# yuansliu/minicom

Measured on AMD Instinct MI355X. Metric: Mreads/s (sketch+index+overlap) on 150bp reads, 1/2/4/8 GPU; bit-exact decompress, higher is better.
Workload: dtype u64

## Files before the change

minicom_amd/csrc/api.hip:

```cpp
#include "mcom_dev.hpp"
#include "../../include/mcom_test.h"
#include <stdarg.h>
#include <stdlib.h>
#include <cxxabi.h>
#include <stdio.h>
#include <string.h>

int mcom_fail(mcom_ctx *ctx, int code, const char *fmt, ...)
{
	char buf[512];
	va_list ap;
	va_start(ap, fmt);
	vsnprintf(buf, sizeof buf, fmt, ap);
	va_end(ap);
	if (ctx) { ctx->err = buf; ctx->pin_wait.clear(); ctx->pin_off = 0; }
	return code;
}

#define MCOM_PIN_BYTES 4096
hipError_t mcom_d2h_async(mcom_ctx *ctx, void *dst, const void *src, size_t bytes)
{
	for (uint32_t q = 0; q < 8; ++q) {
		const mcom_ctx::ScanTotal &t = ctx->scan_last[(ctx->scan_last_at + 7u - q) % 8u];
		if (t.last && t.last == src && t.bytes == bytes && t.gen == ctx->launch_gen) { mcom_ctx::PinWait w{dst, 0, bytes}; w.from = ctx->scan_tot + t.slot; ctx->pin_wait.push_back(w); return hipSuccess; }
// ... 257 lines not shown
extern "C" int mcom_prof_kernels(mcom_ctx *ctx, const char *name, char *buf, size_t cap, size_t *need)
{
	if (!ctx || !name) return MCOM_E_ARG;
	int cls = -1;
	if (!strcmp(name, "*")) cls = -2;
	else if (!strcmp(name, "-")) cls = PROF_COUNT;
	else for (int i = 0; i < PROF_COUNT; ++i) if (!strcmp(name, PROF_NAMES[i])) cls = i;
	if (cls == -1) return mcom_fail(ctx, MCOM_E_ARG, "unknown profiler name %s", name);
	std::map<std::string, uint64_t> out;
	for (const auto &kv : ctx->prof_kernels) if (cls == -2 || kv.first.first == cls) out[prof_kernel_text(ctx, kv.first.second)] += kv.second;
	std::string txt;
	for (const auto &kv : out) { txt += kv.first; txt += '\t'; txt += std::to_string(kv.second); txt += '\n'; }
	if (need) *need = txt.size() + 1;
	if (buf && cap) { size_t m = txt.size() < cap - 1 ? txt.size() : cap - 1; memcpy(buf, txt.data(), m); buf[m] = 0; }
	return MCOM_OK;
}

extern "C" int mcom_prof_read(mcom_ctx *ctx, const char *name, double *total_ms, uint64_t *launches)
{
	if (!ctx || !name) return MCOM_E_ARG;
	prof_collect(ctx);
	for (int i = 0; i < PROF_COUNT; ++i) if (!strcmp(name, PROF_NAMES[i])) {
		if (total_ms) *total_ms = ctx->prof_ms[i];
		if (launches) *launches = ctx->prof_calls[i];
		return MCOM_OK;
	}
	return mcom_fail(ctx, MCOM_E_ARG, "unknown profiler name %s", name);
}

extern "C" uint64_t mcom_counter(const mcom_ctx *ctx, const char *name)
{
	if (!ctx || !name) return 0;
	if (!strcmp(name, "sort_overflow_segments")) return ctx->sort_overflow_segments;
	if (!strcmp(name, "sketch_strings")) return ctx->sketch_strings;
	return 0;
}
extern "C" int mcom_set_segment_capacity(mcom_ctx *ctx, uint32_t records)
{
	if (!ctx || records > 4096) return MCOM_E_ARG;
	ctx->seg_cap = records;
	return MCOM_OK;
}
extern "C" int mcom_set_consensus_capacity(mcom_ctx *ctx, uint32_t members)
{
	if (!ctx) return MCOM_E_ARG;
	ctx->bs_cap = members;
	return MCOM_OK;
}
extern "C" int mcom_set_sketch_kernel(mcom_ctx *ctx, int wave_per_string)
{
	if (!ctx) return MCOM_E_ARG;
	ctx->sketch_wave_only = wave_per_string == 1;
	ctx->sketch_ring64 = wave_per_string == 2;
	ctx->sketch_ring32_only = wave_per_string == 3;
	ctx->sketch_lane_always = wave_per_string >= 2;
	return MCOM_OK;
}
extern "C" int mcom_set_sketch_prefix_bits(mcom_ctx *ctx, int bits)
{
	if (!ctx || bits < 1 || bits > 30) return MCOM_E_ARG;
	ctx->sketch_prefix_bits = bits;
	return MCOM_OK;
}
extern "C" int mcom_set_claim_route(mcom_ctx *ctx, int route)
{
	if (!ctx || route < 0 || route > 3) return MCOM_E_ARG;
	ctx->claim_route = route;
	return MCOM_OK;
}
extern "C" int mcom_claim_fallbacks(const mcom_ctx *ctx) { return ctx ? (int)ctx->claim_fallbacks : 0; }
extern "C" int mcom_set_screen_route(mcom_ctx *ctx, int route)
{
	if (!ctx || route < 0 || route > 2) return MCOM_E_ARG;
	ctx->screen_route = route;
	return MCOM_OK;
}
extern "C" int mcom_screen_fallbacks(const mcom_ctx *ctx) { return ctx ? (int)ctx->screen_fallbacks : 0; }
extern "C" int mcom_set_lookup_route(mcom_ctx *ctx, int route)
{
	if (!ctx || route < 0 || route > 1) return MCOM_E_ARG;
	ctx->lookup_route = route;
	return MCOM_OK;
}
extern "C" int mcom_set_index_capacity(mcom_ctx *ctx, int entries)
{
	if (!ctx) return MCOM_E_ARG;
	ctx->cix_cap_set = entries >= 0; ctx->cix_cap = entries >= 0 ? (uint32_t)entries : 0u;
	return MCOM_OK;
}
```

minicom_amd/csrc/contigs.hip:

```cpp
#include "mcom_dev.hpp"
#include <cstring>
#include <cstdlib>
#include <algorithm>
#include <vector>

#define MAXW 128

__device__ __forceinline__ int nt4_of(uint8_t ch)
{
	const uint8_t u = ch & 0xDF;
	return u == 'A' ? 0 : u == 'C' ? 1 : u == 'G' ? 2 : u == 'T' ? 3 : 4;
}

#define PIECE 128
#define NGRP (PIECE / 64)
#define ERING 256
#define EMASK (ERING - 1)
#define RBCAP 64

__device__ __forceinline__ uint64_t rev_groups64(uint64_t x)
{
	x = __brevll(x);
	return ((x >> 1) & 0x5555555555555555ull) | ((x & 0x5555555555555555ull) << 1);
}
// ... 786 lines not shown
}
__global__ void k_fn_qcounts(const uint32_t *__restrict__ roff, const uint32_t *__restrict__ ord, size_t n, uint32_t *__restrict__ cnt)
{
	const size_t u = (size_t)blockIdx.x * blockDim.x + threadIdx.x;
	if (u > n) return;
	if (u == n) { cnt[u] = 0; return; }
	const uint32_t c = ord ? ord[u] : (uint32_t)u;
	cnt[u] = roff[c + 1] - roff[c];
}
__global__ __launch_bounds__(256) void k_fn_counts_ord(const uint64_t *__restrict__ slots, uint32_t log2cap, uint32_t region, uint32_t bbits,
                                                       const mcom_mm128 *__restrict__ rec, const uint32_t *__restrict__ roff, const uint32_t *__restrict__ ord,
                                                       const uint32_t *__restrict__ qoff, size_t n, uint32_t nq, uint32_t new_lo, uint32_t new_span, int kbits,
                                                       const uint32_t *__restrict__ keymap, uint32_t *__restrict__ hits, uint32_t *__restrict__ first,
                                                       uint64_t *__restrict__ qy)
{
	const size_t u = ((size_t)blockIdx.x * blockDim.x + threadIdx.x) >> 4;
	if (u >= n) return;
	const int lane = threadIdx.x & 15;
	if (u == 0 && lane == 0) hits[nq] = 0;
	const uint32_t c = ord ? ord[u] : (uint32_t)u;
	const uint32_t r0 = roff[c], cnt = roff[c + 1] - r0, q0 = qoff[u];
	const bool old_contig = new_span && !fn_is_new(c, new_lo, new_span);
	for (uint32_t t0 = lane; t0 < cnt; t0 += 64) {
		mcom_mm128 v[4];
#pragma unroll
		for (int u = 0; u < 4; ++u) { const uint32_t t = t0 + 16u * u; if (t < cnt) v[u] = rec[r0 + t]; else { v[u].x = U64MAX; v[u].y = 0; } }
		bool look[4];
#pragma unroll
		for (int u = 0; u < 4; ++u) {
			look[u] = v[u].x != U64MAX;
			if (look[u] && old_contig) { const uint32_t h = fn_key_bit(v[u].x, kbits); look[u] = (keymap[h >> 5] >> (h & 31)) & 1u; }
		}
#pragma unroll
		for (int u = 0; u < 4; ++u) {
			const uint32_t t = t0 + 16u * u;
			if (t >= cnt) break;
			uint32_t s = 0, k = 0;
			if (look[u]) mcom_table_find_any(slots, log2cap, region, bbits, v[u].x, s, k);
			hits[q0 + t] = k;
			if (k) { first[q0 + t] = s; qy[q0 + t] = v[u].y; }
		}
	}
}
__global__ void k_fn_expand(const uint32_t *__restrict__ pair_off, size_t nq, uint32_t *__restrict__ pair_q)
{
	const size_t i = (size_t)blockIdx.x * blockDim.x + threadIdx.x;
	if (i >= nq) return;
	const uint32_t p0 = pair_off[i], p1 = pair_off[i + 1];
	for (uint32_t p = p0; p < p1; ++p) pair_q[p] = (uint32_t)i;
}
__global__ void k_fn_eval(const uint32_t *__restrict__ first, const mcom_mm128 *__restrict__ irec,
                          const mcom_mm128 *__restrict__ q, const uint64_t *__restrict__ qy, const uint32_t *__restrict__ pair_off, const uint32_t *__restrict__ pair_q, uint32_t n_pairs,
                          const uint64_t *__restrict__ cbits, const uint64_t *__restrict__ coff, const uint32_t *__restrict__ clen,
                          int cbthr, uint32_t new_lo, uint32_t new_span, uint32_t *__restrict__ pass)
{
	const uint32_t p = blockIdx.x * blockDim.x + threadIdx.x;
	if (p >= n_pairs) return;
	const uint32_t i = pair_q[p];
	const uint32_t u = p - pair_off[i], s = first[i];
	const uint64_t my = qy ? qy[i] : q[i].y, y = irec[s + u].y;
	const uint32_t ci = (uint32_t)(my >> 32), pos_ori = (uint32_t)my >> 1;
	const uint32_t cj = (uint32_t)(y >> 32), pos = (uint32_t)y >> 1;
	uint32_t ok = 0;
	if (cj != ci && ((my ^ y) & 1) == 0 && (new_span == 0 || fn_is_new(ci, new_lo, new_span) || fn_is_new(cj, new_lo, new_span))) {
		const uint32_t mis = match_pro_packed(cbits + coff[ci], clen[ci], cbits + coff[cj], clen[cj], (int)pos_ori, (int)pos, (uint32_t)cbthr);
		ok = mis <= (uint32_t)cbthr;
	}
	pass[p] = ok;
	if (p == 0) pass[n_pairs] = 0;
}
__global__ void k_fn_emit(const uint32_t *__restrict__ first, const mcom_mm128 *__restrict__ irec,
                          const mcom_mm128 *__restrict__ q, const uint64_t *__restrict__ qy, const uint32_t *__restrict__ pair_off, const uint32_t *__restrict__ pair_q,
                          const uint32_t *__restrict__ pass_pre, uint32_t n_pairs,
                          mcom_mm128 *__restrict__ out)
{
	const uint32_t p = blockIdx.x * blockDim.x + threadIdx.x;
	if (p >= n_pairs) return;
	const uint32_t here = pass_pre[p], nxt = pass_pre[p + 1];
	if (nxt == here) return;
	const uint32_t i = pair_q[p];
	mcom_mm128 v; v.x = qy ? qy[i] : q[i].y; v.y = irec[first[i] + (p - pair_off[i])].y;
	out[here] = v;
}

extern "C" int mcom_find_next_candidates(mcom_ctx *ctx, const mcom_idx *mi, const mcom_mm128 *d_query, size_t n_query,
                                         const uint64_t *d_cbits, const uint64_t *d_coff, const uint32_t *d_clen, int cbthr,
                                         mcom_mm128 *d_out, size_t cap, uint64_t *h_counts)
{
	return mcom_find_next_candidates_new(ctx, mi, d_query, n_query, d_cbits, d_coff, d_clen, cbthr, 0, d_out, cap, h_counts);
}
static int find_next_impl(mcom_ctx *ctx, const mcom_idx *mi, const mcom_mm128 *d_query, size_t n_query, const uint32_t *d_roff, const uint32_t *d_ord, size_t n_contigs,
                          const uint64_t *d_cbits, const uint64_t *d_coff, const uint32_t *d_clen, int cbthr, uint32_t new_lo, uint32_t new_span, uint32_t n_new_hint,
                          mcom_mm128 *d_out, size_t cap, uint64_t *h_counts)
{
	if (!ctx || !mi) return MCOM_E_ARG;
	if (h_counts) { h_counts[0] = h_counts[1] = 0; }
	const bool by_contig = d_roff != nullptr;
	if (by_contig ? n_contigs == 0 : n_query == 0) return MCOM_OK;
	if (!d_query || !d_cbits || !d_coff || !d_clen) return mcom_fail(ctx, MCOM_E_ARG, "null device pointer");
	uint32_t *qoff = nullptr;
	struct FirstGuard { mcom_ctx *c; uint32_t *p; ~FirstGuard() { mcom_dfree_later(c, p); } };
	if (by_contig) {
		if (mcom_dmalloc(&qoff, (n_contigs + 1) * 4) != hipSuccess) return mcom_fail(ctx, MCOM_E_NOMEM, "candidate buffers");
	}
	FirstGuard qoff_guard{ctx, qoff};
	if (by_contig) {
		MCOM_LAUNCH(k_fn_qcounts, dim3((unsigned)((n_contigs + 1 + 255) / 256)), dim3(256), 0, ctx->stream, d_roff, d_ord, n_contigs, qoff);
		MCOM_LAUNCH_CHECK(ctx);
		int rc0 = mcom_scan_u32(ctx, qoff, qoff, n_contigs + 1, nullptr);
		if (rc0) return rc0;
		uint32_t nq = 0;
		MCOM_HIP(ctx, mcom_d2h_async(ctx, &nq, qoff + n_contigs, 4));
		MCOM_HIP(ctx, mcom_stream_sync(ctx));
		n_query = nq;
		if (n_query == 0) return MCOM_OK;
	}
	if (n_query >= (1ull << 31)) return mcom_fail(ctx, MCOM_E_ARG, "too many query minimizers");
	const size_t nq1 = n_query + 1;
	const size_t hit_b = (nq1 * 4 + 255) & ~(size_t)255;
	const size_t scr1_b = (mcom_scan_scratch_elems(nq1) * 4 + 1024 + 255) & ~(size_t)255;
	int kbits = 20;
	while (kbits < 26 && ((uint64_t)1 << kbits) < (uint64_t)n_new_hint * 6 * 16) ++kbits;
	const size_t map_b = new_span ? (size_t)1 << (kbits - 3) : 0;
	int rc = mcom_ws_reserve(ctx, hit_b + scr1_b + map_b);
	if (rc) return rc;
	uint32_t *hits = (uint32_t*)ctx->ws;
	uint32_t *keymap = new_span ? (uint32_t*)((char*)ctx->ws + hit_b + scr1_b) : nullptr;
	uint32_t *first = nullptr, *pair_off = nullptr;
	uint64_t *qy = nullptr;
	if (mcom_dmalloc(&first, nq1 * 4) != hipSuccess) return mcom_fail(ctx, MCOM_E_NOMEM, "candidate buffers");
	FirstGuard first_guard{ctx, first};
	if (mcom_dmalloc(&pair_off, nq1 * 4) != hipSuccess) return mcom_fail(ctx, MCOM_E_NOMEM, "candidate buffers");
	FirstGuard off_guard{ctx, pair_off};
	if (by_contig && mcom_dmalloc(&qy, nq1 * 8) != hipSuccess) return mcom_fail(ctx, MCOM_E_NOMEM, "candidate buffers");
	FirstGuard qy_guard{ctx, (uint32_t*)qy};
	const unsigned qb = (unsigned)((n_query + 255) / 256);
	if (new_span) {
		MCOM_HIP(ctx, hipMemsetAsync(keymap, 0, map_b, ctx->stream));
		if (mi->n) MCOM_LAUNCH(k_fn_newkeys, dim3((unsigned)((mi->n + 255) / 256)), dim3(256), 0, ctx->stream, mi->rec, mi->n, new_lo, new_span, kbits, keymap);
	}
	if (by_contig)
		MCOM_LAUNCH(k_fn_counts_ord, dim3((unsigned)((n_contigs * 16 + 255) / 256)), dim3(256), 0, ctx->stream, mi->tab.slots, mi->tab.log2cap, mi->tab.region, mi->tab.bbits,
		            d_query, d_roff, d_ord, (const uint32_t*)qoff, n_contigs, (uint32_t)n_query, new_lo, new_span, kbits, keymap, hits, first, qy);
	else
		MCOM_LAUNCH(k_fn_counts, dim3(qb), dim3(256), 0, ctx->stream, mi->tab.slots, mi->tab.log2cap, mi->tab.region, mi->tab.bbits, d_query, n_query, new_lo, new_span, kbits, keymap, hits, first);
	MCOM_LAUNCH_CHECK(ctx);
	rc = mcom_scan_u32(ctx, hits, pair_off, nq1, (uint32_t*)((char*)ctx->ws + hit_b));
	if (rc) return rc;
	uint32_t n_pairs = 0;
	MCOM_HIP(ctx, mcom_d2h_async(ctx, &n_pairs, pair_off + n_query, 4));
	MCOM_HIP(ctx, mcom_stream_sync(ctx));
	if (h_counts) h_counts[0] = n_pairs;
	if (n_pairs == 0) return MCOM_OK;
	uint32_t *pass = nullptr, *pair_q = nullptr;
	const size_t scr2_b = (mcom_scan_scratch_elems(n_pairs) * 4 + 1024 + 255) & ~(size_t)255;
	hipError_t e = mcom_dmalloc(&pass, ((size_t)n_pairs + 1) * 4);
	if (e == hipSuccess) e = mcom_dmalloc(&pair_q, (size_t)n_pairs * 4);
	auto cleanup = [&]() { mcom_dfree_later(ctx, pass); mcom_dfree_later(ctx, pair_q); };
	if (e != hipSuccess) { cleanup(); return mcom_fail(ctx, MCOM_E_NOMEM, "candidate buffers: %s", hipGetErrorString(e)); }
	hipError_t e1 = hipSuccess;
	rc = mcom_ws_reserve(ctx, scr2_b);
	if (rc) { cleanup(); return rc; }
	const unsigned pb = (unsigned)(((size_t)n_pairs + 255) / 256);
	{ McomProfScope ps_(ctx, PROF_FIND_NEXT);
	MCOM_LAUNCH(k_fn_expand, dim3(qb), dim3(256), 0, ctx->stream, pair_off, n_query, pair_q);
	MCOM_LAUNCH(k_fn_eval, dim3(pb), dim3(256), 0, ctx->stream, first, mi->rec, d_query, (const uint64_t*)qy, pair_off, pair_q, n_pairs, d_cbits, d_coff, d_clen, cbthr, new_lo, new_span, pass); }
	uint32_t n_pass = 0;
	rc = mcom_scan_u32(ctx, pass, pass, (size_t)n_pairs + 1, (uint32_t*)ctx->ws);
	if (rc) { cleanup(); return rc; }
	hipError_t e1b = mcom_d2h_async(ctx, &n_pass, pass + n_pairs, 4);
	if (e1b == hipSuccess) e1b = mcom_stream_sync(ctx);
	if (e1b != hipSuccess) { cleanup(); return mcom_fail(ctx, MCOM_E_HIP, "candidate scan: %s", hipGetErrorString(e1b)); }
	if (h_counts) h_counts[1] = n_pass;
	if (n_pass > cap) { cleanup(); return mcom_fail(ctx, MCOM_E_OVERFLOW, "%u passing candidates but room for %zu", n_pass, cap); }
	if (n_pass) {
		if (!d_out) { cleanup(); return mcom_fail(ctx, MCOM_E_ARG, "null output pointer"); }
		MCOM_LAUNCH(k_fn_emit, dim3(pb), dim3(256), 0, ctx->stream, first, mi->rec, d_query, (const uint64_t*)qy, pair_off, pair_q, pass, n_pairs, d_out);
		e1 = hipGetLastError();
		if (e1 != hipSuccess) { cleanup(); return mcom_fail(ctx, MCOM_E_HIP, "candidate emit: %s", hipGetErrorString(e1)); }
	}
	cleanup();
	return MCOM_OK;
}
extern "C" int mcom_find_next_candidates_new(mcom_ctx *ctx, const mcom_idx *mi, const mcom_mm128 *d_query, size_t n_query,
                                             const uint64_t *d_cbits, const uint64_t *d_coff, const uint32_t *d_clen, int cbthr, uint32_t n_new,
                                             mcom_mm128 *d_out, size_t cap, uint64_t *h_counts)
{
	return find_next_impl(ctx, mi, d_query, n_query, nullptr, nullptr, 0, d_cbits, d_coff, d_clen, cbthr, 0, n_new, n_new, d_out, cap, h_counts);
}
extern "C" int mcom_find_next_candidates_ord(mcom_ctx *ctx, const mcom_idx *mi, const mcom_mm128 *d_rec, const uint32_t *d_roff, const uint32_t *d_ord, size_t n_contigs,
                                             const uint64_t *d_cbits, const uint64_t *d_coff, const uint32_t *d_clen, int cbthr, uint32_t first_new, uint32_t n_new,
                                             mcom_mm128 *d_out, size_t cap, uint64_t *h_counts)
{
	if (!d_roff) return ctx ? mcom_fail(ctx, MCOM_E_ARG, "null device pointer") : MCOM_E_ARG;
	return find_next_impl(ctx, mi, d_rec, 0, d_roff, d_ord, n_contigs, d_cbits, d_coff, d_clen, cbthr, first_new, n_new ? 0xFFFFFFFFu : 0u, n_new, d_out, cap, h_counts);
}
```

minicom_amd/csrc/mcom_dev.hpp:

```cpp
#pragma once
#include <hip/hip_runtime.h>
#include <stdint.h>
#include <stddef.h>
#include <map>
#include <string>
#include <vector>
#include "../../include/mcom.h"

enum McomProfId { PROF_CLASSIFY_PACK = 0, PROF_SKETCH_READS, PROF_RADIX_PASS, PROF_SKETCH_CONTIGS, PROF_FIND_NEXT,
                  PROF_DICT_BUILD, PROF_REALIGN_WINDOWS, PROF_CONSENSUS, PROF_CINDEX_BUILD, PROF_REALIGN_READS, PROF_COUNT };
struct McomProfSpan { int id; hipEvent_t a, b; };

struct mcom_ctx {
	int device;
	hipStream_t stream;
	std::string err;
	void *ws; size_t ws_bytes;
	int n_cu;
	bool prof_on = false;
	std::vector<McomProfSpan> prof_open;
	double prof_ms[PROF_COUNT] = {0};
	uint64_t prof_calls[PROF_COUNT] = {0};
	int prof_cur = PROF_COUNT;
	std::map<std::pair<int, const void *>, uint64_t> prof_kernels;
	uint32_t seg_cap = 0; uint64_t sort_overflow_segments = 0;
	uint64_t sketch_strings = 0;
	bool cix_cap_set = false; uint32_t cix_cap = 0;
	uint32_t bs_cap = 0;
	bool sketch_wave_only = false;
	bool sketch_lane_always = false;
	bool sketch_ring64 = false, sketch_ring32_only = false; int sketch_prefix_bits = 14;
	unsigned long long *scan_parts = nullptr; uint32_t scan_epoch = 0; volatile unsigned int *poison = nullptr; unsigned int *d_poison = nullptr;
	enum { SCAN_TOTALS = 64 };
	unsigned long long *scan_tot = nullptr, *d_scan_tot = nullptr;
	struct ScanTotal { const void *last; uint32_t bytes, slot, gen; } scan_last[8] = {}; uint32_t scan_last_at = 0, launch_gen = 1;
	int claim_route = 0; uint64_t claim_fallbacks = 0;
	unsigned int *screen_flag = nullptr;
	std::vector<void*> free_later;
	int screen_route = 0; uint64_t screen_fallbacks = 0;
	int lookup_route = 0;
	int verify_hash_bits = 64;
	struct ScreenArgs { const uint64_t *sgbits; size_t n_sg; int L, ininumdict, maxsearch, n_shares, share; } screen_args = {};
	enum { ZPOOL_BYTES = 64 * 1024 };
	unsigned char *zpool = nullptr; size_t zpool_used = 0; int zpool_half = 0;
	struct PinWait { void *dst; size_t off, bytes; const void *from = nullptr; };
	unsigned char *pin = nullptr; size_t pin_off = 0;
	std::vector<PinWait> pin_wait;
};

hipEvent_t mcom_prof_event_get();
void mcom_prof_event_put(hipEvent_t e);
struct McomProfScope {
	mcom_ctx *ctx; int idx;
	McomProfScope(mcom_ctx *c, int id) : ctx(c), idx(-1) {
		if (!c->prof_on) return;
		McomProfSpan s; s.id = id;
		if (!(s.a = mcom_prof_event_get())) return;
		if (!(s.b = mcom_prof_event_get())) { mcom_prof_event_put(s.a); return; }
		(void)hipEventRecord(s.a, c->stream);
		c->prof_open.push_back(s); idx = (int)c->prof_open.size() - 1;
		prev = c->prof_cur; c->prof_cur = id;
	}
	~McomProfScope() { if (idx >= 0) { (void)hipEventRecord(ctx->prof_open[idx].b, ctx->stream); ctx->prof_cur = prev; } }
	int prev = PROF_COUNT;
};
#define MCOM_LAUNCH(kernel, grid, block, lds, stream, ...) do { \
	++ctx->launch_gen; \
	if (ctx->prof_on) ++ctx->prof_kernels[std::make_pair(ctx->prof_cur, (const void*)&kernel)]; \
	hipLaunchKernelGGL(kernel, grid, block, lds, stream, __VA_ARGS__); } while (0)

int mcom_fail(mcom_ctx *ctx, int code, const char *fmt, ...);
hipError_t mcom_d2h_async(mcom_ctx *ctx, void *dst, const void *src, size_t bytes);
hipError_t mcom_stream_sync(mcom_ctx *ctx);
hipError_t mcom_stream_sync_poison(mcom_ctx *ctx, bool *poisoned);
int mcom_ws_reserve(mcom_ctx *ctx, size_t bytes);
void *mcom_zeroed(mcom_ctx *ctx, void *fallback, size_t bytes);
void mcom_ring_flush_slot(mcom_ctx *ctx, uint32_t slot);
unsigned long long *mcom_ring_slot(mcom_ctx *ctx, uint32_t *slot);
void mcom_ring_register(mcom_ctx *ctx, const void *d_result, uint32_t bytes, uint32_t slot);
hipError_t mcom_dmalloc(void **out, size_t bytes);
void mcom_dfree(void *p);
void mcom_dfree_later(mcom_ctx *ctx, void *p);
template <class T> static inline hipError_t mcom_dmalloc(T **out, size_t bytes) { return mcom_dmalloc((void**)out, bytes); }

int mcom_scan_u32(mcom_ctx *ctx, const uint32_t *in, uint32_t *out, size_t n, uint32_t *scratch);
size_t mcom_scan_scratch_elems(size_t n);
int mcom_scan_prepare(mcom_ctx *ctx);
size_t mcom_sort_ws_bytes(size_t n);
int mcom_sort_by_x(mcom_ctx *ctx, mcom_mm128 *d_a, size_t n, int bits, void *ws);
int mcom_sort_by_low_bits(mcom_ctx *ctx, mcom_mm128 *d_a, size_t n, int bits, void *ws);
int mcom_sort_by_low_bits_into_ws(mcom_ctx *ctx, const mcom_mm128 *d_src, mcom_mm128 *d_a, size_t n, int bits, void *ws, mcom_mm128 **d_sorted);
#define MCOM_GROUP_TILE 1280
#define MCOM_GROUP_SCRATCH(n) (4 * ((size_t)(n) / MCOM_GROUP_TILE + 1) + 16)
int mcom_sort_groups_by_x(mcom_ctx *ctx, mcom_mm128 *d_in, mcom_mm128 *d_out, size_t n, const uint64_t *d_goff, size_t ng, int bits, uint32_t *d_scratch);
int mcom_merge_consensus_regions(mcom_ctx *ctx, const uint64_t *d_packed, const uint64_t *d_members, const uint64_t *d_job_off, const uint64_t *d_ref_off,
                                 const uint32_t *d_tile_job, const uint32_t *d_tile_idx, uint32_t n_tiles, int L, uint8_t *d_refs,
                                 const uint32_t *d_reg_lo, const uint32_t *d_reg_hi, const uint32_t *d_tlist);
int mcom_merge_consensus_units(mcom_ctx *ctx, const uint64_t *d_packed, const uint64_t *d_members, const uint64_t *d_job_off, const uint64_t *d_ref_off,
                               const uint32_t *d_ujob, const uint32_t *d_uoff, uint32_t n_units, int L, uint8_t *d_refs,
                               const uint32_t *d_reg_lo, const uint32_t *d_reg_hi, const uint32_t *d_toff, uint32_t n_tiles,
                               unsigned int *d_tflag, uint32_t *d_tlist, uint32_t *h_nlist);
size_t mcom_scan64_scratch_elems(size_t n);
int mcom_scan64(mcom_ctx *ctx, const uint64_t *in, uint64_t *out, size_t n, uint64_t *scratch);
int mcom_device_crc32(mcom_ctx *ctx, const uint8_t *d, uint64_t n, uint32_t *crc_out);

#define MCOM_HIP(ctx, call) do { hipError_t e__ = (call); if (e__ != hipSuccess) \
	return mcom_fail(ctx, MCOM_E_HIP, "%s failed: %s (%s:%d)", #call, hipGetErrorString(e__), __FILE__, __LINE__); } while (0)
#define MCOM_LAUNCH_CHECK(ctx) MCOM_HIP(ctx, hipGetLastError())
#define hipMemsetAsync(...) (++ctx->launch_gen, hipMemsetAsync(__VA_ARGS__))
#define hipMemcpyAsync(dst_, src_, n_, kind_, st_) (((kind_) != hipMemcpyDeviceToHost ? ++ctx->launch_gen : 0u), hipMemcpyAsync(dst_, src_, n_, kind_, st_))

#define U64MAX 0xFFFFFFFFFFFFFFFFull

__device__ __forceinline__ uint64_t mcom_hash64(uint64_t key, uint64_t mask)
{
	key = (~key + (key << 21)) & mask;
	key ^= key >> 24;
	key = (key + (key << 3) + (key << 8)) & mask;
	key ^= key >> 14;
	key = (key + (key << 2) + (key << 4)) & mask;
	key ^= key >> 28;
	key = (key + (key << 31)) & mask;
	return key;
// ... 103 lines not shown
```

minicom_amd/hip.py:

```python
from __future__ import annotations

import ctypes as C
import os
import re

import numpy as np

HERE = os.path.dirname(os.path.abspath(__file__))
MM_DTYPE = np.dtype([("x", "<u8"), ("y", "<u8")])


class McomError(RuntimeError):
    pass


class DecodeSrc(C.Structure):
    _fields_ = [("d_text", C.c_void_p), ("text_bytes", C.c_uint64), ("d_line_start", C.c_void_p), ("verbatim", C.c_int),
                ("d_ref", C.c_void_p), ("ref_bytes", C.c_uint64), ("ref_const", C.c_int),
                ("d_cid", C.c_void_p), ("d_pos", C.c_void_p), ("d_coff", C.c_void_p), ("n_contigs", C.c_uint64),
                ("d_dir", C.c_void_p), ("dir_bytes", C.c_uint64)]


DECODE_F_BOUNDS, DECODE_F_LINE, DECODE_F_DUP, DECODE_F_DEST = 1, 2, 4, 8

# ... 284 lines not shown
        packed = torch.empty((n, W), dtype=torch.int64, device=self.device)
        cls = torch.empty(n, dtype=torch.uint8, device=self.device)
        ncnt = torch.empty(n, dtype=torch.int16, device=self.device)
        nmask = torch.empty((n, (L + 63) // 64), dtype=torch.int64, device=self.device) if want_nmask else None
        rec = self.empty_records(n)
        self._check(self.lib.mcom_process_reads(self._h, self._p(ascii_, torch.uint8), pitch, n, L, k, e, rid0,
                                                self._p(packed), self._p(cls), self._p(ncnt), self._p(nmask), self._p(rec)))
        return {"packed": packed, "cls": cls, "ncnt": ncnt, "nmask": nmask, "rec": rec}

    def process_reads_packed(self, in_packed, in_nmask, L: int, k: int, e: int = 4, rid0: int = 0, in_place: bool = False):
        torch = _torch()
        n = int(in_packed.shape[0])
        packed = in_packed if in_place else torch.empty_like(in_packed)
        nmask = in_nmask if in_place else torch.empty_like(in_nmask)
        cls = torch.empty(n, dtype=torch.uint8, device=self.device)
        ncnt = torch.empty(n, dtype=torch.int16, device=self.device)
        rec = self.empty_records(n)
        self._check(self.lib.mcom_process_reads_packed(self._h, self._p(in_packed, torch.int64), self._p(in_nmask, torch.int64), n, L, k, e, rid0,
                                                       self._p(packed), self._p(cls), self._p(ncnt), self._p(nmask), self._p(rec)))
        return {"packed": packed, "cls": cls, "ncnt": ncnt, "nmask": nmask, "rec": rec}

    def special_reads(self, cls, cap: int = 1 << 20):
        torch = _torch()
        n = int(cls.shape[0])
        out = torch.empty(max(cap, 1), dtype=torch.int64, device=self.device)
        cnt = torch.zeros(2, dtype=torch.int32, device=self.device)
        self._check(self.lib.mcom_special_reads(self._h, self._p(cls, torch.uint8), n, self._p(out), cap, self._p(cnt)))
        self.sync()
        c = int(cnt[0].item())
        return out[: min(c, cap)], c

    def sketch_reads(self, packed, L: int, k: int, rids=None, rid0: int = 0, out=None):
        torch = _torch()
        n = int(rids.shape[0]) if rids is not None else int(packed.shape[0])
        rec = out if out is not None else self.empty_records(n)
        self._check(self.lib.mcom_sketch_reads(self._h, self._p(packed, torch.int64),
                                               self._p(rids, torch.int32) if rids is not None else C.c_void_p(0),
                                               n, L, k, rid0, self._p(rec)))
        return rec

    def hash64(self, kmers, k: int):
        torch = _torch()
        out = torch.empty_like(kmers)
        self._check(self.lib.mcom_hash64_batch(self._h, self._p(kmers, torch.int64), int(kmers.shape[0]), k, self._p(out)))
        return out

    def encode_byte(self, rows, cg, contig, pos, dirs, L: int):
        torch = _torch()
        n = int(rows.shape[0])
        ok = torch.empty(max(n, 1), dtype=torch.uint8, device=self.device)
        self._check(self.lib.mcom_encode_byte(self._h, self._p(rows, torch.int64), self._p(cg["cbits"]), self._p(cg["coff"]), self._p(contig, torch.int32),
                                              self._p(pos, torch.int32), self._p(dirs, torch.uint8), n, L, self._p(ok)))
        return ok[:n]

    def radix_sort_128x(self, rec):
        torch = _torch()
        self._check(self.lib.mcom_radix_sort_128x(self._h, self._p(rec, torch.int64), int(rec.shape[0])))
        return rec

    def counter(self, name: str) -> int:
        self.lib.mcom_counter.restype = C.c_uint64; self.lib.mcom_counter.argtypes = [C.c_void_p, C.c_char_p]
        return int(self.lib.mcom_counter(self._h, name.encode()))

    def set_segment_capacity(self, records: int):
        self.lib.mcom_set_segment_capacity.restype = C.c_int; self.lib.mcom_set_segment_capacity.argtypes = [C.c_void_p, C.c_uint32]
        self._check(self.lib.mcom_set_segment_capacity(self._h, records))

    def set_index_capacity(self, entries: int):
        self.lib.mcom_set_index_capacity.restype = C.c_int; self.lib.mcom_set_index_capacity.argtypes = [C.c_void_p, C.c_int]
        self._check(self.lib.mcom_set_index_capacity(self._h, entries))

    def set_sketch_kernel(self, wave_per_string):
        self.lib.mcom_set_sketch_kernel.restype = C.c_int; self.lib.mcom_set_sketch_kernel.argtypes = [C.c_void_p, C.c_int]
        self._check(self.lib.mcom_set_sketch_kernel(self._h, int(wave_per_string)))

    def set_sketch_prefix_bits(self, bits: int):
        self.lib.mcom_set_sketch_prefix_bits.restype = C.c_int; self.lib.mcom_set_sketch_prefix_bits.argtypes = [C.c_void_p, C.c_int]
        self._check(self.lib.mcom_set_sketch_prefix_bits(self._h, bits))

    def set_claim_route(self, route: int):
        self.lib.mcom_set_claim_route.restype = C.c_int; self.lib.mcom_set_claim_route.argtypes = [C.c_void_p, C.c_int]
        self._check(self.lib.mcom_set_claim_route(self._h, route))

    def claim_fallbacks(self) -> int:
        self.lib.mcom_claim_fallbacks.restype = C.c_int; self.lib.mcom_claim_fallbacks.argtypes = [C.c_void_p]
        return int(self.lib.mcom_claim_fallbacks(self._h))

    def set_screen_route(self, route: int):
        self.lib.mcom_set_screen_route.restype = C.c_int; self.lib.mcom_set_screen_route.argtypes = [C.c_void_p, C.c_int]
        self._check(self.lib.mcom_set_screen_route(self._h, route))

    def screen_fallbacks(self) -> int:
        self.lib.mcom_screen_fallbacks.restype = C.c_int; self.lib.mcom_screen_fallbacks.argtypes = [C.c_void_p]
        return int(self.lib.mcom_screen_fallbacks(self._h))

    def set_consensus_capacity(self, members: int):
        self.lib.mcom_set_consensus_capacity.restype = C.c_int; self.lib.mcom_set_consensus_capacity.argtypes = [C.c_void_p, C.c_uint32]
        self._check(self.lib.mcom_set_consensus_capacity(self._h, members))

    def sort_group(self, rec, L: int, k_orig: int, kmer: int, b: int = 14):
        torch = _torch()
        n = int(rec.shape[0])
        srt = self.empty_records(n)
        singles = torch.empty(max(n, 1), dtype=torch.int32, device=self.device)
        sord = torch.empty(max(n, 1), dtype=torch.int32, device=self.device)
        members = torch.empty(max(n, 1), dtype=torch.int64, device=self.device)
        goff = torch.empty(n // 2 + 2, dtype=torch.int32, device=self.device)
        cnt = (C.c_uint64 * 4)()
        self._check(self.lib.mcom_sort_group(self._h, self._p(rec, torch.int64), n, L, k_orig, kmer, b, self._p(srt),
                                             self._p(singles), self._p(sord), self._p(members), self._p(goff), cnt))
        nv, ns, ng, nm = (int(x) for x in cnt)
        return {"sorted": srt, "n_valid": nv, "singles": singles[:ns], "single_ord": sord[:ns], "members": members[:nm], "group_off": goff[:ng + 1] if n else goff[:0],
                "n_groups": ng}

    def upload_contigs(self, refs):
        torch = _torch()
        lens = np.array([len(r) for r in refs], dtype=np.int64)
        off = np.concatenate([[0], np.cumsum(lens)]).astype(np.int64)
        words = (2 * lens + 63) // 64 + 1
        coff = np.concatenate([[0], np.cumsum(words)[:-1]]).astype(np.int64) if len(refs) else np.zeros(0, np.int64)
        total = int(words.sum())
        seq = torch.from_numpy(np.frombuffer(b"".join(refs) + b"\0", dtype=np.uint8).copy()).to(self.device)
        d_off = torch.from_numpy(off).to(self.device)
        d_coff = torch.from_numpy(coff).to(self.device)
        d_clen = torch.from_numpy(lens.astype(np.int32)).to(self.device)
        cbits = torch.zeros(total + 1, dtype=torch.int64, device=self.device)
        self._check(self.lib.mcom_pack_contigs(self._h, self._p(seq), self._p(d_off), self._p(d_coff), len(refs), total, self._p(cbits)))
        return {"seq": seq, "off": d_off, "coff": d_coff, "clen": d_clen, "cbits": cbits, "n": len(refs), "lens": lens}

    def unpack_contigs(self, cbits, coff, off, n: int, byte_lo: int, byte_hi: int, seq):
        self.lib.mcom_unpack_contigs.restype = C.c_int
        self.lib.mcom_unpack_contigs.argtypes = [C.c_void_p] * 4 + [C.c_uint32, C.c_uint64, C.c_uint64, C.c_void_p]
        self._check(self.lib.mcom_unpack_contigs(self._h, self._p(cbits), self._p(coff), self._p(off), n, byte_lo, byte_hi, self._p(seq)))

    def sketch_contigs(self, seq, off, n: int, w: int, k: int, max_per_contig: int = 0, ids=None):
        torch = _torch()
        moff = torch.empty(n + 1, dtype=torch.int32, device=self.device)
        total = C.c_uint64(0)
        cap = max(1024, 2 * n * (max_per_contig if max_per_contig else 4))
        while True:
            out = self.empty_records(cap)
            rc = self.lib.mcom_sketch_contigs(self._h, self._p(seq), self._p(off), self._p(ids), n, w, k, max_per_contig,
                                              self._p(moff), self._p(out), cap, C.byref(total))
            if rc == -4:
                cap = int(total.value)
                continue
            self._check(rc)
            return moff, out[: int(total.value)]

    def idx_build(self, rec, k: int, b: int = 14):
        return Index(self, rec, k, b)

    def radix_sort_128x_ref_order(self, rec):
        torch = _torch()
        self._check(self.lib.mcom_radix_sort_128x_ref_order(self._h, self._p(rec, torch.int64), int(rec.shape[0])))
        return rec

    def match_pro(self, cg, a, pa, b, pb):
        torch = _torch()
        n = int(a.shape[0])
        out = torch.empty(n, dtype=torch.int32, device=self.device)
        self._check(self.lib.mcom_match_pro(self._h, self._p(cg["cbits"]), self._p(cg["coff"]), self._p(cg["clen"]),
                                            self._p(a, torch.int32), self._p(pa, torch.int32), self._p(b, torch.int32), self._p(pb, torch.int32), n, self._p(out)))
        return out

    def find_next_candidates(self, idx, query, cg, cbthr: int):
# ... 1077 lines not shown
```

Baseline: 553.6.

## Compact passing candidates per workgroup during eval and gather via per-block scan

The candidate eval kernel now writes passing pairs directly into a per-workgroup staging buffer using ballot-based compaction, and emits one count per workgroup instead of one flag per pair. The prefix scan then runs over workgroup counts rather than over all pairs, and a gather kernel copies staged results to the output. This removes the full-length per-pair scan and the emit kernel's re-read of the query and index records. The price is an extra staging buffer of n_pairs records. Optional grouped variants (4/8/16 lanes per pair) are selectable, and the default is one lane per pair.

Measured after the change: 562.4 (median of 6 runs). +1.6%, better.

```diff
diff --git a/minicom_amd/csrc/api.hip b/minicom_amd/csrc/api.hip
--- a/minicom_amd/csrc/api.hip
+++ b/minicom_amd/csrc/api.hip
@@ -363,6 +363,12 @@
 	ctx->lookup_route = route;
 	return MCOM_OK;
 }
+extern "C" int mcom_set_eval_route(mcom_ctx *ctx, int route)
+{
+	if (!ctx || (route != 0 && route != 1 && route != 4 && route != 8 && route != 16)) return MCOM_E_ARG;
+	ctx->eval_route = route;
+	return MCOM_OK;
+}
 extern "C" int mcom_set_index_capacity(mcom_ctx *ctx, int entries)
 {
 	if (!ctx) return MCOM_E_ARG;
diff --git a/minicom_amd/csrc/contigs.hip b/minicom_amd/csrc/contigs.hip
--- a/minicom_amd/csrc/contigs.hip
+++ b/minicom_amd/csrc/contigs.hip
@@ -892,6 +892,88 @@
 	mcom_mm128 v; v.x = qy ? qy[i] : q[i].y; v.y = irec[first[i] + (p - pair_off[i])].y;
 	out[here] = v;
 }
+static const int FN_EVAL_G = 1;
+template <int G>
+__global__ __launch_bounds__(256) void k_fn_eval_grp(const uint32_t *__restrict__ first, const mcom_mm128 *__restrict__ irec,
+                          const mcom_mm128 *__restrict__ q, const uint64_t *__restrict__ qy, const uint32_t *__restrict__ pair_off, const uint32_t *__restrict__ pair_q, uint32_t n_pairs,
+                          const uint64_t *__restrict__ cbits, const uint64_t *__restrict__ coff, const uint32_t *__restrict__ clen,
+                          int cbthr, uint32_t new_lo, uint32_t new_span, mcom_mm128 *__restrict__ stage, uint32_t *__restrict__ wg_cnt)
+{
+	constexpr uint32_t PPW = 256 / G;
+	__shared__ uint32_t wave_cnt[4];
+	const uint32_t sub = threadIdx.x & (G - 1);
+	const size_t p = (size_t)blockIdx.x * PPW + threadIdx.x / G;
+	uint64_t my = 0, y = 0;
+	bool ok = false;
+	if (p < n_pairs) {
+		const uint32_t i = pair_q[p];
+		const uint32_t u = (uint32_t)p - pair_off[i], s = first[i];
+		my = qy ? qy[i] : q[i].y; y = irec[s + u].y;
+		const uint32_t ci = (uint32_t)(my >> 32), pos_ori = (uint32_t)my >> 1;
+		const uint32_t cj = (uint32_t)(y >> 32), pos = (uint32_t)y >> 1;
+		if (cj != ci && ((my ^ y) & 1) == 0 && (new_span == 0 || fn_is_new(ci, new_lo, new_span) || fn_is_new(cj, new_lo, new_span))) {
+			const uint64_t *A = cbits + coff[ci], *B = cbits + coff[cj];
+			const long lenA = (long)clen[ci], lenB = (long)clen[cj];
+			const long d = (long)(int)pos_ori - (long)(int)pos;
+			const long lo = d > 0 ? d : 0;
+			long hi = lenB + d; if (hi > lenA) hi = lenA;
+			const long nb_all = hi - lo;
+			const uint32_t nw = nb_all > 0 ? (uint32_t)((nb_all + 31) >> 5) : 0u;
+			const long ahead = d > 0 ? d : -d;
+			const uint64_t *S = (d > 0 ? A : B) + (ahead >> 5), *T = d > 0 ? B : A;
+			const int sh = (int)((2 * ahead) & 63);
+			const uint32_t thr = (uint32_t)cbthr;
+			uint32_t mis = 0;
+			for (uint32_t k0 = 0; k0 < nw; k0 += G) {
+				const uint32_t k = k0 + sub;
+				const bool have = k < nw;
+				uint64_t ws = 0, wt = 0;
+				if (have) { ws = S[k]; wt = T[k]; }
+				uint64_t x = ws;
+				if (sh) {
+					uint64_t nx = 0;
+					if (G > 1) nx = __shfl_down((unsigned long long)ws, 1, G);
+					if (have && (sub == G - 1 || k + 1 == nw)) nx = S[k + 1];
+					x = (ws >> sh) | (nx << (64 - sh));
+				}
+				x ^= wt;
+				x = (x | (x >> 1)) & 0x5555555555555555ull;
+				if (k + 1 == nw) { const long nb = nb_all - 32 * (long)k; if (nb < 32) x &= (1ull << (2 * nb)) - 1; }
+				uint32_t c = have ? (uint32_t)__popcll(x) : 0u;
+#pragma unroll
+				for (int o = G / 2; o; o >>= 1) c += (uint32_t)__shfl_xor((int)c, o, G);
+				mis += c;
+				if (mis > thr) break;
+			}
+			ok = mis <= thr;
+		}
+	}
+	const bool lead = ok && sub == 0;
+	const unsigned long long bal = __ballot(lead);
+	const uint32_t lane = threadIdx.x & 63, wv = threadIdx.x >> 6;
+	if (lane == 0) wave_cnt[wv] = (uint32_t)__popcll(bal);
+	__syncthreads();
+	uint32_t before = 0, tot = 0;
+#pragma unroll
+	for (uint32_t w = 0; w < 4; ++w) { const uint32_t c = wave_cnt[w]; if (w < wv) before += c; tot += c; }
+	if (lead) {
+		mcom_mm128 v; v.x = my; v.y = y;
+		stage[(size_t)blockIdx.x * PPW + before + (uint32_t)__popcll(bal & ((1ull << lane) - 1))] = v;
+	}
+	if (threadIdx.x == 0) {
+		wg_cnt[blockIdx.x] = tot;
+		if (blockIdx.x == 0) wg_cnt[gridDim.x] = 0;
+	}
+}
+template <int G>
+__global__ void k_fn_gather(const mcom_mm128 *__restrict__ stage, const uint32_t *__restrict__ wg_off, uint32_t n_wg, size_t cap, mcom_mm128 *__restrict__ out)
+{
+	constexpr uint32_t PPW = 256 / G, LPR = G == 1 ? 32 : 8;
+	const size_t t = (size_t)blockIdx.x * blockDim.x + threadIdx.x, w = t / LPR;
+	if (w >= n_wg) return;
+	const uint32_t o0 = wg_off[w], n = wg_off[w + 1] - o0;
+	for (uint32_t r = (uint32_t)(t % LPR); r < n; r += LPR) { const size_t o = (size_t)o0 + r; if (o < cap) out[o] = stage[w * PPW + r]; }
+}
 
 extern "C" int mcom_find_next_candidates(mcom_ctx *ctx, const mcom_idx *mi, const mcom_mm128 *d_query, size_t n_query,
                                          const uint64_t *d_cbits, const uint64_t *d_coff, const uint32_t *d_clen, int cbthr,
@@ -962,30 +1044,43 @@
 	MCOM_HIP(ctx, mcom_stream_sync(ctx));
 	if (h_counts) h_counts[0] = n_pairs;
 	if (n_pairs == 0) return MCOM_OK;
+	const int G = ctx->eval_route == 1 ? 0 : ctx->eval_route ? ctx->eval_route : FN_EVAL_G;
+	const size_t n_cnt = G ? ((size_t)n_pairs + 256 / G - 1) / (256 / G) : (size_t)n_pairs;
 	uint32_t *pass = nullptr, *pair_q = nullptr;
-	const size_t scr2_b = (mcom_scan_scratch_elems(n_pairs) * 4 + 1024 + 255) & ~(size_t)255;
-	hipError_t e = mcom_dmalloc(&pass, ((size_t)n_pairs + 1) * 4);
+	mcom_mm128 *stage = nullptr;
+	const size_t scr2_b = (mcom_scan_scratch_elems(n_cnt) * 4 + 1024 + 255) & ~(size_t)255;
+	hipError_t e = mcom_dmalloc(&pass, (n_cnt + 1) * 4);
 	if (e == hipSuccess) e = mcom_dmalloc(&pair_q, (size_t)n_pairs * 4);
-	auto cleanup = [&]() { mcom_dfree_later(ctx, pass); mcom_dfree_later(ctx, pair_q); };
+	if (e == hipSuccess && G) e = mcom_dmalloc(&stage, (size_t)n_pairs * sizeof(mcom_mm128));
+	auto cleanup = [&]() { mcom_dfree_later(ctx, pass); mcom_dfree_later(ctx, pair_q); mcom_dfree_later(ctx, stage); };
 	if (e != hipSuccess) { cleanup(); return mcom_fail(ctx, MCOM_E_NOMEM, "candidate buffers: %s", hipGetErrorString(e)); }
 	hipError_t e1 = hipSuccess;
 	rc = mcom_ws_reserve(ctx, scr2_b);
 	if (rc) { cleanup(); return rc; }
-	const unsigned pb = (unsigned)(((size_t)n_pairs + 255) / 256);
+	const unsigned pb = (unsigned)(G ? n_cnt : ((size_t)n_pairs + 255) / 256);
+#define FN_EVAL_GRP(GG) MCOM_LAUNCH((k_fn_eval_grp<GG>), dim3(pb), dim3(256), 0, ctx->stream, first, mi->rec, d_query, (const uint64_t*)qy, pair_off, pair_q, n_pairs, \
+	                                d_cbits, d_coff, d_clen, cbthr, new_lo, new_span, stage, pass)
 	{ McomProfScope ps_(ctx, PROF_FIND_NEXT);
 	MCOM_LAUNCH(k_fn_expand, dim3(qb), dim3(256), 0, ctx->stream, pair_off, n_query, pair_q);
-	MCOM_LAUNCH(k_fn_eval, dim3(pb), dim3(256), 0, ctx->stream, first, mi->rec, d_query, (const uint64_t*)qy, pair_off, pair_q, n_pairs, d_cbits, d_coff, d_clen, cbthr, new_lo, new_span, pass); }
+	if (G == 1) FN_EVAL_GRP(1); else if (G == 4) FN_EVAL_GRP(4); else if (G == 8) FN_EVAL_GRP(8); else if (G == 16) FN_EVAL_GRP(16);
+	else MCOM_LAUNCH(k_fn_eval, dim3(pb), dim3(256), 0, ctx->stream, first, mi->rec, d_query, (const uint64_t*)qy, pair_off, pair_q, n_pairs, d_cbits, d_coff, d_clen, cbthr, new_lo, new_span, pass); }
+#undef FN_EVAL_GRP
 	uint32_t n_pass = 0;
-	rc = mcom_scan_u32(ctx, pass, pass, (size_t)n_pairs + 1, (uint32_t*)ctx->ws);
+	rc = mcom_scan_u32(ctx, pass, pass, n_cnt + 1, (uint32_t*)ctx->ws);
 	if (rc) { cleanup(); return rc; }
-	hipError_t e1b = mcom_d2h_async(ctx, &n_pass, pass + n_pairs, 4);
+	hipError_t e1b = mcom_d2h_async(ctx, &n_pass, pass + n_cnt, 4);
 	if (e1b == hipSuccess) e1b = mcom_stream_sync(ctx);
 	if (e1b != hipSuccess) { cleanup(); return mcom_fail(ctx, MCOM_E_HIP, "candidate scan: %s", hipGetErrorString(e1b)); }
 	if (h_counts) h_counts[1] = n_pass;
 	if (n_pass > cap) { cleanup(); return mcom_fail(ctx, MCOM_E_OVERFLOW, "%u passing candidates but room for %zu", n_pass, cap); }
 	if (n_pass) {
 		if (!d_out) { cleanup(); return mcom_fail(ctx, MCOM_E_ARG, "null output pointer"); }
-		MCOM_LAUNCH(k_fn_emit, dim3(pb), dim3(256), 0, ctx->stream, first, mi->rec, d_query, (const uint64_t*)qy, pair_off, pair_q, pass, n_pairs, d_out);
+		const unsigned gb = (unsigned)((n_cnt * (G == 1 ? 32 : 8) + 255) / 256);
+		if (G == 1) MCOM_LAUNCH((k_fn_gather<1>), dim3(gb), dim3(256), 0, ctx->stream, stage, pass, (uint32_t)n_cnt, cap, d_out);
+		else if (G == 4) MCOM_LAUNCH((k_fn_gather<4>), dim3(gb), dim3(256), 0, ctx->stream, stage, pass, (uint32_t)n_cnt, cap, d_out);
+		else if (G == 8) MCOM_LAUNCH((k_fn_gather<8>), dim3(gb), dim3(256), 0, ctx->stream, stage, pass, (uint32_t)n_cnt, cap, d_out);
+		else if (G == 16) MCOM_LAUNCH((k_fn_gather<16>), dim3(gb), dim3(256), 0, ctx->stream, stage, pass, (uint32_t)n_cnt, cap, d_out);
+		else MCOM_LAUNCH(k_fn_emit, dim3(pb), dim3(256), 0, ctx->stream, first, mi->rec, d_query, (const uint64_t*)qy, pair_off, pair_q, pass, n_pairs, d_out);
 		e1 = hipGetLastError();
 		if (e1 != hipSuccess) { cleanup(); return mcom_fail(ctx, MCOM_E_HIP, "candidate emit: %s", hipGetErrorString(e1)); }
 	}
diff --git a/minicom_amd/csrc/mcom_dev.hpp b/minicom_amd/csrc/mcom_dev.hpp
--- a/minicom_amd/csrc/mcom_dev.hpp
+++ b/minicom_amd/csrc/mcom_dev.hpp
@@ -39,6 +39,7 @@
 	std::vector<void*> free_later;
 	int screen_route = 0; uint64_t screen_fallbacks = 0;
 	int lookup_route = 0;
+	int eval_route = 0;
 	int verify_hash_bits = 64;
 	struct ScreenArgs { const uint64_t *sgbits; size_t n_sg; int L, ininumdict, maxsearch, n_shares, share; } screen_args = {};
 	enum { ZPOOL_BYTES = 64 * 1024 };
diff --git a/minicom_amd/hip.py b/minicom_amd/hip.py
--- a/minicom_amd/hip.py
+++ b/minicom_amd/hip.py
@@ -390,6 +390,10 @@
         self.lib.mcom_set_claim_route.restype = C.c_int; self.lib.mcom_set_claim_route.argtypes = [C.c_void_p, C.c_int]
         self._check(self.lib.mcom_set_claim_route(self._h, route))
 
+    def set_eval_route(self, route: int):
+        self.lib.mcom_set_eval_route.restype = C.c_int; self.lib.mcom_set_eval_route.argtypes = [C.c_void_p, C.c_int]
+        self._check(self.lib.mcom_set_eval_route(self._h, route))
+
     def claim_fallbacks(self) -> int:
         self.lib.mcom_claim_fallbacks.restype = C.c_int; self.lib.mcom_claim_fallbacks.argtypes = [C.c_void_p]
         return int(self.lib.mcom_claim_fallbacks(self._h))
```
